# bdina9/qat-vit

Measured on AMD Instinct MI355X. Metric: images/sec QAT student step (fwd+bwd+allreduce), higher is better.
Workload: dtype f32 (emulated: int8 MFMA for grid x grid products; forward float operands as fp16 hi+lo pairs; backward gradients as ONE fp16 plane scaled per tensor - 2^-12 per element, <= 4e-4 relative L2 per stage against the fp32 reference, bf16-pair fallback on overflow; fp32 / exact-integer accumulate)

## Files before the change

include/qatvit.h:

```cpp
#ifndef QATVIT_H
#define QATVIT_H

#include <stdint.h>

#ifdef __cplusplus
extern "C" {
#endif
#if defined(__GNUC__) || defined(__clang__)
#pragma GCC visibility push(default)
#endif

#define QATVIT_ABI_VERSION 4

int qatvit_abi_version(void);
const char* qatvit_last_error(void);
const char* qatvit_target_arch(void);

int64_t qatvit_fq_workspace_bytes(int64_t channels);
int qatvit_fq_forward(const float* x, float* y, uint8_t* mask_bits,
                      float* running_min, float* running_max, float* scale, int32_t* zero_point,
                      const int64_t* observer_on, const int64_t* fake_quant_on,
                      float averaging_const, int32_t qmin, int32_t qmax,
                      int64_t channels, int64_t inner, int32_t per_channel, int32_t symmetric,
                      void* workspace, void* stream);
// ... 75 lines not shown
    const void* P; const void* Q; const uint32_t* lut; const float* s1; const float* s2; float* C; const float* W; const float* w_scale; const int32_t* w_zp; float* dbias;
    const float* row_div; int32_t N, Kw, ldp, ldq, ldc;
};
int64_t qatvit_gemm_tn_stream_scratch_bytes(void);
int qatvit_gemm_tn_stream_dy16(int32_t mode, const struct qatvit_tn_item* items, int32_t n, int32_t M, int32_t center, int32_t w_per_channel, int32_t w_qmin, int32_t w_qmax,
                               float* scratch, int64_t scratch_bytes, void* stream);

int32_t qatvit_attn_padded_tokens(int32_t T);
int qatvit_attn_forward(const float* qkv, const float* qp, int32_t qmin, int32_t qmax, int32_t B, int32_t T, int32_t H,
                        int32_t D, void* O_hi, void* O_lo, float* lse, void* stream);
int qatvit_attn_forward_f16(const float* qkv, const float* qp, int32_t qmin, int32_t qmax, int32_t B, int32_t T, int32_t H,
                            int32_t D, void* O_hi, void* O_lo, float* lse, void* O16_hi, void* O16_lo, float* o16_scale, void* qkv_codes,
                            void* qkv_mask, void* stream);
int qatvit_attn_backward(const float* qkv, const float* qp, int32_t qmin, int32_t qmax, int32_t B, int32_t T, int32_t H,
                         int32_t D, const void* O_hi, const void* O_lo, const float* lse, float* delta, const float* dO,
                         void* dqkv_hi, void* dqkv_lo, const float* col_scale, const void* qkv_codes, const void* qkv_mask, void* stream);
int qatvit_attn_backward_live(const float* qkv, const float* qp, int32_t qmin, int32_t qmax, int32_t B, int32_t T, int32_t H,
                              int32_t D, const void* O_hi, const void* O_lo, const float* lse, float* delta, const float* dO,
                              void* dqkv_hi, void* dqkv_lo, const float* col_scale, const void* qkv_codes, const void* qkv_mask,
                              int32_t live_q_tiles, int32_t dO_cls, void* stream);

int qatvit_rows_gather(const void* tall, void* compact, int32_t rows, int32_t T, int32_t width, int64_t stride, void* stream);
int qatvit_rows_scatter(const void* compact, void* tall, int32_t rows, int32_t T, int32_t width, void* stream);

typedef struct qatvit_cfg {
    int32_t batch, img_size, patch_size, in_chans;
    int32_t embed_dim, depth, num_heads, mlp_hidden, num_classes;
    int32_t act_qmin, act_qmax;
    int32_t w_qmin, w_qmax;
    int32_t w_per_channel;
    float averaging_const;
    float ln_eps;
} qatvit_cfg;

typedef struct qatvit_fq {
    float* min_val;
    float* max_val;
    float* scale;
    int32_t* zero_point;
    const int64_t* observer_on;
    const int64_t* fake_quant_on;
} qatvit_fq;

int32_t qatvit_student_num_params(const qatvit_cfg* cfg);
int32_t qatvit_student_num_act_fq(const qatvit_cfg* cfg);
int32_t qatvit_student_num_weight_fq(const qatvit_cfg* cfg);
// ... 127 lines not shown
```

qat-vit_amd/csrc/capi.hip:

```cpp
#include <stdarg.h>
#include <stdlib.h>
#include <string.h>

#include "../../include/qatvit.h"
#include "qv_common.h"
#include "qv_kernels.h"

namespace qv {
static thread_local char g_err[512] = "";
void set_error(const char* fmt, ...) {
    va_list ap;
    va_start(ap, fmt);
    vsnprintf(g_err, sizeof(g_err), fmt, ap);
    va_end(ap);
}

static bool knob(const char* name) {
    const char* v = getenv(name);
    return !v || atoi(v) != 0;
}
const Knobs& knobs() {
    static const Knobs k{knob("QATVIT_I8"), knob("QATVIT_F16"), knob("QATVIT_FC2_CODES"), knob("QATVIT_FC1_BITS"), knob("QATVIT_FC2W_CODES"),
                         knob("QATVIT_WBATCH"), knob("QATVIT_ATTN_CODES"), knob("QATVIT_QKV_2PASS"), knob("QATVIT_LNB_FUSE"), knob("QATVIT_QP_LATE"),
                         knob("QATVIT_TN_STREAM"), knob("QATVIT_TN_Q8"), knob("QATVIT_ATTN_BWD_FUSED"), knob("QATVIT_F16_STRIP"), knob("QATVIT_I8_STRIP"), knob("QATVIT_LN_STRIP"),
                         knob("QATVIT_CLS_BWD")};
    return k;
}
}

using namespace qv;

extern "C" {

int qatvit_abi_version(void) { return QATVIT_ABI_VERSION; }
const char* qatvit_last_error(void) { return qv::g_err; }
const char* qatvit_target_arch(void) { return "gfx950"; }

int64_t qatvit_fq_workspace_bytes(int64_t channels) {
    if (channels < 1) channels = 1;
    return channels * (2 * (int64_t)sizeof(uint32_t) + 4 * (int64_t)sizeof(float));
}

int qatvit_fq_forward(const float* x, float* y, uint8_t* mask_bits, float* running_min, float* running_max, float* scale,
                      int32_t* zero_point, const int64_t* observer_on, const int64_t* fake_quant_on, float averaging_const,
                      int32_t qmin, int32_t qmax, int64_t channels, int64_t inner, int32_t per_channel, int32_t symmetric,
                      void* workspace, void* stream) {
    QV_CHECK_ARG(x && y && running_min && running_max && scale && zero_point && observer_on && fake_quant_on && workspace,
                 "qatvit_fq_forward: null pointer argument");
// ... 443 lines not shown
                     ((uintptr_t)mix & 3) == 0 && ((uintptr_t)erase & 3) == 0,
                 "qatvit_image_batch_rrc_erase: misaligned pointer");
    if (launch_image_batch_rrc_erase(data, index, B, N, S, D, windows, table, rrc, mix, erase, out, (hipStream_t)stream)) return 1;
    QV_CHECK_LAUNCH("qatvit_image_batch_rrc_erase");
    return 0;
}

int qatvit_rows_gather(const void* tall, void* compact, int32_t rows, int32_t T, int32_t width, int64_t stride, void* stream) {
    RowMoveTab t;
    t.n = 1; t.m[0] = RowMove{tall, compact, stride, width};
    if (launch_rows_gather(t, rows, T, (hipStream_t)stream)) return 1;
    QV_CHECK_LAUNCH("qatvit_rows_gather");
    return 0;
}

int qatvit_rows_scatter(const void* compact, void* tall, int32_t rows, int32_t T, int32_t width, void* stream) {
    RowMoveTab t;
    t.n = 1; t.m[0] = RowMove{compact, tall, width, width};
    if (launch_rows_scatter(t, rows, T, (hipStream_t)stream)) return 1;
    QV_CHECK_LAUNCH("qatvit_rows_scatter");
    return 0;
}

}
```

qat-vit_amd/csrc/elt.hip:

```cpp
#include <stdlib.h>

#include <algorithm>

#include "qv_common.h"
#include "qv_device.h"
#include "qv_kernels.h"
#include "qv_qparams.h"

namespace qv {

struct QP { float s, inv, zp, on; };
__device__ inline QP load_qp(const float* qp) { return QP{qp[0], qp[1], qp[2], qp[3]}; }
__device__ inline float fqv(float x, const QP& q, float fqmin, float fqmax, bool& in) {
    const float t = rintf(x * q.inv) + q.zp;
    in = (t >= fqmin && t <= fqmax) || q.on == 0.f;
    const float y = (fminf(fmaxf(t, fqmin), fqmax) - q.zp) * q.s;
    return q.on != 0.f ? y : x;
}
__device__ inline float fqi(float x, const QP& q, float fqmin, float fqmax) {
    return fminf(fmaxf(rintf(x * q.inv) + q.zp, fqmin), fqmax) - q.zp;
}

__device__ inline void store_split4(__bf16* hi, __bf16* lo, int64_t off, float a, float b, float c, float d) {
    uint2 h, l;
// ... 412 lines not shown
    __syncthreads();
    const int lane = threadIdx.x & 63, wave = threadIdx.x >> 6;
    for (int c = wave; c < C; c += 4) {
        float acc = 0.f;
        for (int k = lane; k < D; k += 64) acc += sh[k] * (float)wq[(int64_t)c * D + k];
        acc = wave_sum(acc);
        if (lane == 0) {
            const float v = acc * (q.s * w_scale[w_per_channel ? c : 0]) + bias[c];
            logits_pre[(int64_t)b * C + c] = v;
            stat_atomic(stats, stat_slots, v, v);
        }
    }
}

__global__ void k_logits_fq(const float* __restrict__ pre, const float* __restrict__ qp, int qmin, int qmax, float* __restrict__ out, int n) {
    const QP q = load_qp(qp);
    const int i = blockIdx.x * blockDim.x + threadIdx.x;
    if (i < n) {
        bool in;
        out[i] = fqv(pre[i], q, qmin, qmax, in);
    }
}

__global__ __launch_bounds__(256) void k_head_bwd(const float* __restrict__ dlogits, const float* __restrict__ logits_pre, const float* __restrict__ qp_logits,
                                                  int qmin, int qmax, const float* __restrict__ hq, const float* __restrict__ qp_norm,
                                                  const __bf16* __restrict__ wq, const float* __restrict__ W, const float* __restrict__ w_scale,
                                                  const int32_t* __restrict__ w_zp, int w_per_channel, int w_qmin, int w_qmax,
                                                  float* __restrict__ dW, float* __restrict__ dbias, float* __restrict__ dh, int B, int D, int C) {
    const QP ql = load_qp(qp_logits);
    const int kch = (D + 63) / 64;
    if ((int)blockIdx.x < C * kch) {
        const int c = blockIdx.x / kch, k = (blockIdx.x % kch) * 64 + (threadIdx.x & 63), grp = threadIdx.x >> 6;
        const float s_norm = qp_norm[0];
        const int ci = w_per_channel ? c : 0;
        const float inv = __fdiv_rn(1.0f, w_scale[ci]), fzp = (float)w_zp[ci];
        float acc = 0.f, dbacc = 0.f;
        const int bper = (B + 3) / 4, b_lo = grp * bper, b_hi = min(B, b_lo + bper);
        if (k < D) {
            for (int b = b_lo; b < b_hi; ++b) {
                bool in;
                fqv(logits_pre[(int64_t)b * C + c], ql, qmin, qmax, in);
                const float dl = in ? dlogits[(int64_t)b * C + c] : 0.f;
                acc += dl * hq[(int64_t)b * D + k];
                dbacc += dl;
            }
        }
        __shared__ float sacc[4][64], sdb[4];
        sacc[grp][threadIdx.x & 63] = acc;
        if ((threadIdx.x & 63) == 0) sdb[grp] = dbacc;
        __syncthreads();
        if (grp == 0 && k < D) {
            const float tot = ((sacc[0][threadIdx.x] + sacc[1][threadIdx.x]) + sacc[2][threadIdx.x]) + sacc[3][threadIdx.x];
            const float t = rintf(W[(int64_t)c * D + k] * inv) + fzp;
            const bool win = t >= (float)w_qmin && t <= (float)w_qmax;
            dW[(int64_t)c * D + k] = win ? tot * s_norm : 0.f;
            if (k == 0) dbias[c] = ((sdb[0] + sdb[1]) + sdb[2]) + sdb[3];
        }
    } else {
        const int b = blockIdx.x - C * kch;
        for (int k = threadIdx.x; k < D; k += blockDim.x) {
            float acc = 0.f;
            for (int c = 0; c < C; ++c) {
                bool in;
                fqv(logits_pre[(int64_t)b * C + c], ql, qmin, qmax, in);
                const float dl = in ? dlogits[(int64_t)b * C + c] : 0.f;
                acc += dl * (float)wq[(int64_t)c * D + k] * w_scale[w_per_channel ? c : 0];
            }
            dh[(int64_t)b * D + k] = acc;
        }
    }
}

__global__ __launch_bounds__(64) void k_embed_bwd(const float* __restrict__ dx0, const float* __restrict__ Y0, const float* __restrict__ qp,
                                                  int qmin, int qmax, float* __restrict__ dpos, float* __restrict__ dcls,
                                                  __bf16* __restrict__ dY0_hi, __bf16* __restrict__ dY0_lo, int B, int T, int D) {
    const QP q = load_qp(qp);
    const int d4 = D / 4;
    const int64_t n4 = (int64_t)T * d4;
    constexpr int UNR = 16;
    for (int64_t i = blockIdx.x * (int64_t)blockDim.x + threadIdx.x; i < n4; i += (int64_t)gridDim.x * blockDim.x) {
        const int t = (int)(i / d4), c = (int)(i % d4) * 4;
        const int ty = t > 0 ? t - 1 : 0;
        float4 acc = make_float4(0.f, 0.f, 0.f, 0.f);
        for (int b0 = 0; b0 < B; b0 += UNR) {
            float4 g[UNR], y[UNR];
#pragma unroll
            for (int u = 0; u < UNR; ++u) {
                const int b = b0 + u < B ? b0 + u : B - 1;
                g[u] = *reinterpret_cast<const float4*>(dx0 + ((int64_t)b * T + t) * D + c);
                y[u] = *reinterpret_cast<const float4*>(Y0 + ((int64_t)b * (T - 1) + ty) * D + c);
            }
#pragma unroll
            for (int u = 0; u < UNR; ++u) { pin4(g[u]); pin4(y[u]); }
#pragma unroll
            for (int u = 0; u < UNR; ++u) {
                if (b0 + u < B) {
                    acc.x += g[u].x; acc.y += g[u].y; acc.z += g[u].z; acc.w += g[u].w;
                    if (t > 0) {
                        bool i0, i1, i2, i3;
                        fqv(y[u].x, q, qmin, qmax, i0); fqv(y[u].y, q, qmin, qmax, i1); fqv(y[u].z, q, qmin, qmax, i2); fqv(y[u].w, q, qmin, qmax, i3);
                        store_split4(dY0_hi, dY0_lo, ((int64_t)(b0 + u) * (T - 1) + (t - 1)) * D + c, i0 ? g[u].x : 0.f, i1 ? g[u].y : 0.f,
                                     i2 ? g[u].z : 0.f, i3 ? g[u].w : 0.f);
                    }
                }
            }
        }
        *reinterpret_cast<float4*>(dpos + (int64_t)t * D + c) = acc;
        if (t == 0) *reinterpret_cast<float4*>(dcls + c) = acc;
    }
}

__device__ inline void wquant_body(const float* __restrict__ W, const float* __restrict__ qp, int per_channel, int qmin, int qmax,
                                   __bf16* __restrict__ wq, __bf16* __restrict__ wqT, int N, int K, int bx, int by,
                                   int8_t* __restrict__ w8 = nullptr, int32_t* __restrict__ wsum = nullptr, _Float16* __restrict__ w16 = nullptr,
                                   int8_t* __restrict__ w8f = nullptr, int64_t wT16_gap = 0,
                                   bool wT16_frag = false) {
    __shared__ float tile[32][33];
    const int tx = threadIdx.x & 31, ty = threadIdx.x >> 5;
    const int n0 = by * 32, k0 = bx * 32;
#pragma unroll
    for (int i = 0; i < 4; ++i) {
        const int n = n0 + ty + 8 * i, k = k0 + tx;
        float v = 0.f;
        if (n < N && k < K) {
            const QP q = load_qp(qp + 4 * (per_channel ? n : 0));
            v = q.on != 0.f ? fqi(W[(int64_t)n * K + k], q, qmin, qmax) : W[(int64_t)n * K + k];
            wq[(int64_t)n * K + k] = (__bf16)v;
            if (w8) w8[(int64_t)n * K + k] = (int8_t)v;
            if (w16) w16[(int64_t)n * K + k] = (_Float16)v;
            if (w8f) w8f[w8f_offset(n, k, K)] = (int8_t)v;
        }
// ... 11 lines not shown
        char* const wT16f = (wT16_gap && wT16_frag) ? reinterpret_cast<char*>(wqT) + 2 * wT16_gap : nullptr;
#pragma unroll
        for (int i = 0; i < 4; ++i) {
            const int k = k0 + ty + 8 * i, n = n0 + tx;
            if (n < N && k < K) {
                wqT[(int64_t)k * N + n] = (__bf16)tile[tx][ty + 8 * i];
                if (wT16) wT16[(int64_t)k * N + n] = (_Float16)tile[tx][ty + 8 * i];
                if (wT16f) *reinterpret_cast<_Float16*>(wT16f + w8f_offset(k, 2 * n, 2 * N)) = (_Float16)tile[tx][ty + 8 * i];
            }
        }
    }
}
__global__ __launch_bounds__(256) void k_wquant(const float* __restrict__ W, const float* __restrict__ qp, int per_channel, int qmin, int qmax,
                                                __bf16* __restrict__ wq, __bf16* __restrict__ wqT, int N, int K) {
    wquant_body(W, qp, per_channel, qmin, qmax, wq, wqT, N, K, blockIdx.x, blockIdx.y);
}
__global__ __launch_bounds__(256) void k_w_quant_all(const WQuantTab t) {
    int wi = 0;
    while (wi + 1 < t.n && (int)blockIdx.x >= t.blk0[wi + 1]) ++wi;
    const int b = blockIdx.x - t.blk0[wi], kt = (t.K[wi] + 31) / 32;
    wquant_body(t.W[wi], t.qp[wi], t.per_channel, t.qmin, t.qmax, reinterpret_cast<__bf16*>(t.wq[wi]), reinterpret_cast<__bf16*>(t.wqT[wi]), t.N[wi],
                t.K[wi], b % kt, b / kt, reinterpret_cast<int8_t*>(t.w8[wi]), t.wsum[wi], reinterpret_cast<_Float16*>(t.w16[wi]),
                reinterpret_cast<int8_t*>(t.w8f[wi]), t.wT16 ? wT16_gap_bytes(t.N[wi], t.K[wi]) : 0, ((t.wT16f_mask >> wi) & 1ull) != 0);
}
static_assert(sizeof(WQuantTab) <= 4096, "WQuantTab travels as a kernel argument");
__global__ __launch_bounds__(256) void k_w8_fragment_order(const int8_t* __restrict__ B8, int8_t* __restrict__ B8f, int N, int K) {
    const int64_t i = blockIdx.x * (int64_t)blockDim.x + threadIdx.x;
    if (i >= (int64_t)N * K) return;
    B8f[w8f_offset((int)(i / K), (int)(i % K), K)] = B8[i];
}
int launch_w8_fragment_order(const void* B8, void* B8f, int N, int K, hipStream_t st) {
    if (N < 48 || N % 48 != 0 || K % 64 != 0 || !B8 || !B8f) { set_error("w8_fragment_order: need N %% 48 == 0, K %% 64 == 0 (N=%d K=%d)", N, K); return 1; }
    k_w8_fragment_order<<<cdiv((int64_t)N * K, 256), 256, 0, st>>>(reinterpret_cast<const int8_t*>(B8), reinterpret_cast<int8_t*>(B8f), N, K);
    return 0;
}

int launch_img_patches(const float* img, void* out_bf16, const float* qp, int qmin, int qmax, int B, int C, int H, int W, int P, hipStream_t st,
                       void* out8, int center) {
    if (P % 8 != 0 || H % P != 0 || W % P != 0) { set_error("img_patches: patch %d must be a multiple of 8 and divide %dx%d", P, H, W); return 1; }
    const int64_t n8 = (int64_t)B * C * H * W / 8;
    k_img_patches<<<flat_grid(n8), 256, 0, st>>>(img, reinterpret_cast<__bf16*>(out_bf16), qp, qmin, qmax, B, C, H, W, P, reinterpret_cast<int8_t*>(out8),
                                                 center);
    return 0;
}

int launch_resid_fq_lnstats(int mode, const float* x_prev, const float* Y, const float* qpY, int qmin, int qmax, const float* cls, const float* pos,
// ... 72 lines not shown
    const int nv = (D + 255) / 256;
    if (acc) { if (nv == 1) QV_LNB(1, 1); else if (nv == 2) QV_LNB(1, 2); else QV_LNB(1, 3); }
    else { if (nv == 1) QV_LNB(0, 1); else if (nv == 2) QV_LNB(0, 2); else QV_LNB(0, 3); }
#undef QV_LNB
    return 0;
}

int launch_head_fwd(const float* x, const float* mean, const float* rstd, const float* gamma, const float* beta, const float* qp_norm, int qmin,
                    int qmax, const void* wq, const float* w_scale, int w_per_channel, const float* bias, float* hq, float* logits_pre,
                    uint32_t* stats, int stat_slots, int B, int D, int T, int C, hipStream_t st) {
    k_head_fwd<<<B, 256, D * sizeof(float), st>>>(x, mean, rstd, gamma, beta, qp_norm, qmin, qmax, reinterpret_cast<const __bf16*>(wq), w_scale,
                                                   w_per_channel, bias, hq, logits_pre, stats, stat_slots, D, T, C);
    return 0;
}

int launch_logits_fq(const float* pre, const float* qp, int qmin, int qmax, float* out, int n, hipStream_t st) {
    k_logits_fq<<<cdiv(n, 256), 256, 0, st>>>(pre, qp, qmin, qmax, out, n);
    return 0;
}

int launch_head_bwd(const float* dlogits, const float* logits_pre, const float* qp_logits, int qmin, int qmax, const float* hq, const float* qp_norm,
                    const void* wq, const float* W, const float* w_scale, const int32_t* w_zp, int w_per_channel, int w_qmin, int w_qmax, float* dW,
                    float* dbias, float* dh, int B, int D, int C, hipStream_t st) {
    k_head_bwd<<<C * ((D + 63) / 64) + B, 256, 0, st>>>(dlogits, logits_pre, qp_logits, qmin, qmax, hq, qp_norm, reinterpret_cast<const __bf16*>(wq), W, w_scale, w_zp,
                                      w_per_channel, w_qmin, w_qmax, dW, dbias, dh, B, D, C);
    return 0;
}

int launch_embed_bwd(const float* dx0, const float* Y0, const float* qp, int qmin, int qmax, float* dpos, float* dcls, void* dY0_hi, void* dY0_lo,
                     int B, int T, int D, hipStream_t st) {
    k_embed_bwd<<<(int)cdiv((int64_t)T * (D / 4), 64), 64, 0, st>>>(dx0, Y0, qp, qmin, qmax, dpos, dcls, reinterpret_cast<__bf16*>(dY0_hi),
                                                                  reinterpret_cast<__bf16*>(dY0_lo), B, T, D);
    return 0;
}

__global__ void k_zero_i32(int32_t* p, int64_t n) {
    for (int64_t i = blockIdx.x * (int64_t)blockDim.x + threadIdx.x; i < n; i += (int64_t)gridDim.x * blockDim.x) p[i] = 0;
}
int launch_zero_i32(int32_t* p, int64_t n, hipStream_t st) {
    k_zero_i32<<<(int)cdiv(n, 256) > 1024 ? 1024 : (int)cdiv(n, 256), 256, 0, st>>>(p, n);
    return 0;
}
__global__ __launch_bounds__(256) void k_rows_gather(const RowMoveTab t, int rows, int T) {
    const RowMove m = t.m[blockIdx.y];
    const int wpr = m.width / 4;
    const int64_t tall = (int64_t)T * (m.stride / 4);
    const uint32_t* __restrict__ src = reinterpret_cast<const uint32_t*>(m.src);
    uint32_t* __restrict__ dst = reinterpret_cast<uint32_t*>(m.dst);
    const int total = rows * wpr;
    for (int i = blockIdx.x * 256 + threadIdx.x; i < total; i += gridDim.x * 256) {
        const int b = i / wpr, j = i - b * wpr;
        dst[i] = src[b * tall + j];
    }
}
// ... 18 lines not shown
        const int unit = scatter ? 16 : 4;
        const bool ok = m.src && m.dst && m.width >= unit && m.width % unit == 0 && m.stride % unit == 0 && (scatter ? m.stride == m.width : m.stride >= m.width) &&
                        (int64_t)rows * (scatter ? T : 1) * (m.width / unit) < (1ll << 31) &&
                        (reinterpret_cast<uintptr_t>(m.src) | reinterpret_cast<uintptr_t>(m.dst)) % unit == 0;
        if (!ok) { set_error("%s: tensor %d: width %d, stride %lld (bytes; need %% %d == 0%s, aligned bases, < 2^31 units)", who, k, m.width, (long long)m.stride, unit,
                             scatter ? " and stride == width" : ""); return 1; }
    }
    return 0;
}
int launch_rows_gather(const RowMoveTab& t, int rows, int T, hipStream_t st) {
    if (rows_check("rows_gather", t, rows, T, false)) return 1;
    int64_t most = 0;
    for (int k = 0; k < t.n; ++k) most = std::max<int64_t>(most, (int64_t)rows * (t.m[k].width / 4));
    k_rows_gather<<<dim3(std::min(cdiv(most, 256), 512), t.n), 256, 0, st>>>(t, rows, T);
    return 0;
}
int launch_rows_scatter(const RowMoveTab& t, int rows, int T, hipStream_t st) {
    if (rows_check("rows_scatter", t, rows, T, true)) return 1;
    int64_t most = 0;
    for (int k = 0; k < t.n; ++k) most = std::max<int64_t>(most, (int64_t)rows * T * (t.m[k].width / 16));
    k_rows_scatter<<<dim3(std::min(cdiv(most, 256 * 4), 4096), t.n), 256, 0, st>>>(t, rows, T);
    return 0;
}
int launch_w_quant_all(WQuantTab& t, hipStream_t st) {
    int b = 0;
    for (int i = 0; i < t.n; ++i) {
        t.blk0[i] = b;
        b += (int)(cdiv(t.K[i], 32) * cdiv(t.N[i], 32));
    }
    t.blk0[t.n] = b;
    k_w_quant_all<<<b, 256, 0, st>>>(t);
    return 0;
}
int launch_wquant(const float* W, const float* qp, int per_channel, int qmin, int qmax, void* wq, void* wqT, int N, int K, hipStream_t st) {
    dim3 grid(cdiv(K, 32), cdiv(N, 32));
    k_wquant<<<grid, 256, 0, st>>>(W, qp, per_channel, qmin, qmax, reinterpret_cast<__bf16*>(wq), reinterpret_cast<__bf16*>(wqT), N, K);
    return 0;
}

}
```

qat-vit_amd/csrc/qv_common.h:

```cpp
#pragma once
#include <hip/hip_runtime.h>
#include <stdint.h>
#include <stdio.h>

namespace qv {

constexpr int kWave = 64;

void set_error(const char* fmt, ...);

struct Knobs {
    bool i8;
    bool f16;
    bool fc2_codes;
    bool fc1_bits;
    bool fc2w_codes;
    bool wbatch;
    bool attn_codes;
    bool qkv_2pass;
    bool lnb_fuse;
    bool qp_late;
    bool tn_stream;
    bool tn_q8;
    bool attn_bwd_fused;
    bool f16_strip;
    bool i8_strip;
    bool ln_strip;
    bool cls_bwd;
};
const Knobs& knobs();

#define QV_CHECK_ARG(cond, ...)                 \
    do {                                        \
        if (!(cond)) {                          \
            qv::set_error(__VA_ARGS__);         \
            return 1;                           \
        }                                       \
    } while (0)

#define QV_CHECK_LAUNCH(name)                                                     \
    do {                                                                          \
        hipError_t e_ = hipGetLastError();                                        \
        if (e_ != hipSuccess) {                                                   \
            qv::set_error("%s: launch failed: %s", name, hipGetErrorString(e_));  \
            return 2;                                                             \
        }                                                                         \
    } while (0)

__host__ __device__ inline uint32_t f2ord(float f) {
    uint32_t u = __builtin_bit_cast(uint32_t, f);
// ... 80 lines not shown
```

qat-vit_amd/csrc/qv_kernels.h:

```cpp
#pragma once
#include <hip/hip_runtime.h>
#include <stdint.h>

namespace qv {

int launch_fq_forward(const float* x, float* y, uint8_t* mask_bits, float* running_min, float* running_max, float* scale,
                      int32_t* zero_point, const int64_t* observer_on, const int64_t* fake_quant_on, float c, int qmin, int qmax,
                      int64_t channels, int64_t inner, bool per_channel, bool symmetric, void* workspace, hipStream_t st);
int launch_fq_backward(const float* dy, const uint8_t* mask_bits, float* dx, int64_t n, hipStream_t st);

int launch_ln_forward(const float* x, const float* gamma, const float* beta, float* y, float* mean, float* rstd, int64_t rows,
                      int64_t dim, float eps, hipStream_t st);
int launch_ln_backward(const float* dy, const float* x, const float* gamma, const float* mean, const float* rstd, float* dx,
                       float* dgamma, float* dbeta, int64_t rows, int64_t dim, hipStream_t st);

int launch_kd_ce_loss(const float* student, const float* teacher, const int64_t* labels, int64_t batch, int64_t classes, float kd_temp,
                      float kd_alpha, float label_smoothing, float* out3, float* dlogits, hipStream_t st);
int launch_kd_ce_loss_table(const float* student, const float* table, int64_t table_rows, const int64_t* index, const int64_t* labels, int64_t batch,
                            int64_t classes, float kd_temp, float kd_alpha, float label_smoothing, float* out3, float* dlogits, hipStream_t st);
int launch_kd_ce_loss_mix(const float* student, const float* teacher, const float* table, int64_t table_rows, const int64_t* index,
                          const int64_t* labels, const int32_t* mix, int64_t batch, int64_t classes, float kd_temp, float kd_alpha,
                          float label_smoothing, float* out3, float* dlogits, hipStream_t st);

int launch_minmax(const float* x, int64_t channels, int64_t inner, int per_channel, uint32_t* ws, int nslots, hipStream_t st);
// ... 131 lines not shown
int launch_logits_fq(const float* pre, const float* qp, int qmin, int qmax, float* out, int n, hipStream_t st);
int launch_head_bwd(const float* dlogits, const float* logits_pre, const float* qp_logits, int qmin, int qmax, const float* hq, const float* qp_norm,
                    const void* wq, const float* W, const float* w_scale, const int32_t* w_zp, int w_per_channel, int w_qmin, int w_qmax, float* dW,
                    float* dbias, float* dh, int B, int D, int C, hipStream_t st);
int launch_embed_bwd(const float* dx0, const float* Y0, const float* qp, int qmin, int qmax, float* dpos, float* dcls, void* dY0_hi, void* dY0_lo,
                     int B, int T, int D, hipStream_t st);
constexpr int kMaxW = 52;
struct WObsTab { const float* W[kMaxW]; uint32_t* ws[kMaxW]; int N[kMaxW], K[kMaxW], blk0[kMaxW + 1]; int n, per_channel, nslots; };
struct WQpTab {
    uint32_t* ws[kMaxW]; float* rmin[kMaxW]; float* rmax[kMaxW]; float* scale[kMaxW]; int32_t* zp[kMaxW]; float* qp[kMaxW];
    const int64_t* obs_on[kMaxW]; const int64_t* fq_on[kMaxW]; int N[kMaxW], blk0[kMaxW + 1]; int n, per_channel, nslots, qmin, qmax; float c;
};
struct WQuantTab {
    const float* W[kMaxW]; const float* qp[kMaxW]; void* wq[kMaxW]; void* wqT[kMaxW]; void* w8[kMaxW]; int32_t* wsum[kMaxW];
    void* w16[kMaxW];
    void* w8f[kMaxW];
    int N[kMaxW], K[kMaxW], blk0[kMaxW + 1]; int n, per_channel, qmin, qmax;
    int wT16;
    unsigned long long wT16f_mask;
};
__host__ __device__ inline int64_t wT16_gap_bytes(int N, int K) { return ((int64_t)N * K * 2 + 255) & ~(int64_t)255; }
int launch_w_observe_all(WObsTab& t, hipStream_t st);
int launch_w_qparams_all(WQpTab& t, hipStream_t st);
int launch_w_quant_all(WQuantTab& t, hipStream_t st);
int launch_zero_i32(int32_t* p, int64_t n, hipStream_t st);
struct ObsFoldEntry {
    uint32_t* ws; float* rmin; float* rmax; float* scale; int32_t* zp; const int64_t* obs_on; const int64_t* fq_on;
    int32_t channels, nslots, symmetric, qmin, qmax, blk0;
};
int launch_obs_fold(const ObsFoldEntry* tab, int n, int nblocks, float c, hipStream_t st);
int launch_wquant(const float* W, const float* qp, int per_channel, int qmin, int qmax, void* wq, void* wqT, int N, int K, hipStream_t st);

constexpr int kDyHdrWords = 64, kDySlotWords = 256, kDyAmaxStride = 32, kDyAmaxSlots = 8;
inline int64_t dy16_state_bytes(int nslots) { return 4ll * (kDyHdrWords + (int64_t)nslots * kDySlotWords); }
int launch_dy16_begin(uint32_t* state, int nslots, const float* dlogits, int n_dlogits, hipStream_t st);
int launch_dy16_set_mirror(uint32_t* state, void* host_pinned, hipStream_t st);
int launch_dy16_end(uint32_t* state, int nslots, int check_overflow, hipStream_t st);
int launch_absmax_bf16(const void* hi, int64_t n, uint32_t* amax, hipStream_t st);
int launch_q8_to_bf16int(const void* q8, const float* qp, int center, void* plane, int64_t n, hipStream_t st);
int launch_f16int_to_bf16int(void* plane, int64_t n, hipStream_t st);

int attn_padded_tokens(int T);
int launch_attn_fwd(const float* qkv, const float* qp, int qmin, int qmax, int B, int T, int H, int D, void* O_hi, void* O_lo, float* lse,
                    hipStream_t st, void* O16_hi = nullptr, void* O16_lo = nullptr, float* o16_scale = nullptr, void* codes = nullptr,
                    void* cmask = nullptr);
int launch_attn_bwd(const float* qkv, const float* qp, int qmin, int qmax, int B, int T, int H, int D, const void* O_hi, const void* O_lo,
                    const float* lse, float* delta, const float* dO, void* dqkv_hi, void* dqkv_lo, const float* col_scale, hipStream_t st,
// ... 65 lines not shown
```

qat-vit_amd/native.py:

```python
from __future__ import annotations

import ctypes
import os
import subprocess
from ctypes import c_char_p, c_double, c_float, c_int, c_int32, c_int64, c_void_p

_HERE = os.path.dirname(os.path.abspath(__file__))
LIB_PATH = os.path.join(_HERE, "libqatvit.so")
CSRC = os.path.join(_HERE, "csrc")
_lib = None

SIGNATURES = {
    "qatvit_abi_version": (c_int, []),
    "qatvit_last_error": (c_char_p, []),
    "qatvit_target_arch": (c_char_p, []),
    "qatvit_fq_workspace_bytes": (c_int64, [c_int64]),
    "qatvit_fq_forward": (c_int, [c_void_p] * 9 + [c_float, c_int32, c_int32, c_int64, c_int64, c_int32, c_int32, c_void_p, c_void_p]),
    "qatvit_fq_backward": (c_int, [c_void_p, c_void_p, c_void_p, c_int64, c_void_p]),
    "qatvit_ln_forward": (c_int, [c_void_p] * 6 + [c_int64, c_int64, c_float, c_void_p]),
    "qatvit_ln_backward": (c_int, [c_void_p] * 8 + [c_int64, c_int64, c_void_p]),
    "qatvit_kd_ce_loss": (c_int, [c_void_p, c_void_p, c_void_p, c_int64, c_int64, c_float, c_float, c_float, c_void_p, c_void_p, c_void_p]),
    "qatvit_kd_ce_loss_table": (c_int, [c_void_p, c_void_p, c_int64, c_void_p, c_void_p, c_int64, c_int64, c_float, c_float, c_float, c_void_p, c_void_p, c_void_p]),
    "qatvit_kd_ce_loss_mix": (c_int, [c_void_p, c_void_p, c_void_p, c_int64, c_void_p, c_void_p, c_void_p, c_int64, c_int64, c_float, c_float, c_float,
                                      c_void_p, c_void_p, c_void_p]),
# ... 3 lines not shown
    "qatvit_optim_adamw_ema": (c_int, [c_void_p] * 8 + [c_int32, c_int64] + [c_double] * 5 + [c_int64, c_double, c_void_p, c_void_p]),
    "qatvit_optim_adamw_groups_ema": (c_int, [c_void_p] * 9 + [c_int32, c_int64, c_void_p, c_int32, c_double, c_void_p, c_void_p]),
    "qatvit_optim_ema": (c_int, [c_void_p] * 5 + [c_int32, c_int64, c_double, c_void_p]),
    "qatvit_optim_swap": (c_int, [c_void_p] * 5 + [c_int32, c_int64, c_void_p]),
    "qatvit_gemm_nt": (c_int, [c_void_p] * 4 + [c_int32] * 6 + [c_void_p] * 6),
    "qatvit_gemm_nt_f16": (c_int, [c_void_p] * 4 + [c_int32] * 6 + [c_void_p] * 6),
    "qatvit_gemm_nt_i8_minmax": (c_int, [c_void_p] * 4 + [c_int32] * 6 + [c_void_p] * 6),
    "qatvit_w8_fragment_order": (c_int, [c_void_p, c_void_p, c_int32, c_int32, c_void_p]),
    "qatvit_i8_strip": (c_int, [c_int32] + [c_void_p] * 4 + [c_int32] * 5 + [c_void_p] * 6 + [c_int32, c_int32, c_void_p, c_void_p, c_int32] + [c_void_p] * 4),
    "qatvit_ln_apply_quant8": (c_int, [c_void_p] * 6 + [c_int32, c_int32, c_void_p, c_int32, c_int64, c_int32, c_void_p]),
    "qatvit_i8_strip_ln": (c_int, [c_void_p] * 5 + [c_int32, c_int32] + [c_void_p] * 4 + [c_int32] * 5 + [c_void_p] * 5),
    "qatvit_gemm_nt_codes": (c_int, [c_void_p] * 4 + [c_int32] * 6 + [c_void_p] * 6),
    "qatvit_gemm_nt_i8": (c_int, [c_void_p] * 4 + [c_int32, c_void_p] + [c_int32] * 6 + [c_void_p] * 6),
    "qatvit_gemm_tn_scratch_bytes": (c_int64, []),
    "qatvit_gemm_tn": (c_int, [c_void_p] * 5 + [c_int32] * 6 + [c_void_p] * 4 + [c_int32] * 3 + [c_void_p] * 3 + [c_int64, c_void_p]),
    "qatvit_gemm_tn_codes": (c_int, [c_void_p] * 5 + [c_int32] * 6 + [c_void_p] * 4 + [c_int32] * 3 + [c_void_p] * 3 + [c_int64, c_void_p]),
    "qatvit_gemm_nt_dy16": (c_int, [c_void_p] * 3 + [c_int32] * 6 + [c_void_p] * 3),
    "qatvit_gemm_tn_dy16": (c_int, [c_void_p] * 6 + [c_int32] * 6 + [c_void_p] * 5 + [c_int32] * 3 + [c_void_p] * 3 + [c_int64, c_void_p]),
    "qatvit_gemm_tn_q8_dy16": (c_int, [c_void_p] * 3 + [c_int32, c_void_p] + [c_int32] * 6 + [c_void_p] * 4 + [c_int32] * 3 + [c_void_p] * 3 + [c_int64, c_void_p]),
    "qatvit_gemm_tn_stream_scratch_bytes": (c_int64, []),
    "qatvit_gemm_tn_stream_dy16": (c_int, [c_int32, c_void_p, c_int32, c_int32, c_int32, c_int32, c_int32, c_int32, c_void_p, c_int64, c_void_p]),
    "qatvit_rows_gather": (c_int, [c_void_p, c_void_p, c_int32, c_int32, c_int32, c_int64, c_void_p]),
    "qatvit_rows_scatter": (c_int, [c_void_p, c_void_p, c_int32, c_int32, c_int32, c_void_p]),
    "qatvit_attn_padded_tokens": (c_int32, [c_int32]),
    "qatvit_attn_forward": (c_int, [c_void_p, c_void_p] + [c_int32] * 6 + [c_void_p] * 4),
    "qatvit_attn_forward_f16": (c_int, [c_void_p, c_void_p] + [c_int32] * 6 + [c_void_p] * 9),
    "qatvit_attn_backward": (c_int, [c_void_p, c_void_p] + [c_int32] * 6 + [c_void_p] * 11),
    "qatvit_attn_backward_live": (c_int, [c_void_p, c_void_p] + [c_int32] * 6 + [c_void_p] * 10 + [c_int32, c_int32, c_void_p]),
    "qatvit_student_num_params": (c_int32, [c_void_p]),
    "qatvit_student_num_act_fq": (c_int32, [c_void_p]),
    "qatvit_student_num_weight_fq": (c_int32, [c_void_p]),
    "qatvit_student_workspace_bytes": (c_int64, [c_void_p]),
    "qatvit_student_init": (c_int, [c_void_p, c_void_p, c_void_p]),
    "qatvit_student_forward": (c_int, [c_void_p] * 8),
    "qatvit_student_backward": (c_int, [c_void_p] * 7 + [c_int32, c_int32, c_void_p]),
    "qatvit_student_forward_stages": (c_int, [c_void_p] * 7 + [c_int32, c_int32, c_int32, c_void_p]),
    "qatvit_student_forward_part": (c_int, [c_void_p] * 5 + [c_int32, c_int32, c_int32, c_void_p]),
    "qatvit_student_backward_stages": (c_int, [c_void_p] * 7 + [c_int32, c_int32, c_int32, c_void_p]),
    "qatvit_student_tensor_offset": (c_int64, [c_void_p, c_char_p, c_int32]),
    "qatvit_student_dy16_supported": (c_int32, [c_void_p]),
    "qatvit_student_ln_in_strip": (c_int32, [c_void_p, c_int32]),
    "qatvit_student_dy16_to_pair": (c_int, [c_void_p, c_void_p, c_void_p]),
    "qatvit_student_dy16_set_mirror": (c_int, [c_void_p, c_void_p, c_void_p, c_void_p]),
    "qatvit_teacher_workspace_bytes": (c_int64, [c_void_p]),
    "qatvit_teacher_forward": (c_int, [c_void_p] * 8),
    "qatvit_teacher_forward_f16": (c_int, [c_void_p, c_void_p, c_void_p, c_int32, c_void_p, c_void_p, c_void_p, c_void_p]),
# ... 132 lines not shown
```

Baseline: 16640.

## Split batch reductions across thread groups and add vectorized weight-quant kernel

The head-backward kernel now splits its batch reduction across 16 wave groups instead of 4 and unrolls the per-sample loads by four. The embed-backward kernel splits the batch across 8 groups per 32 items and combines the partial sums in shared memory, which gives more parallelism along B. A new vectorized weight-quantization kernel handles 64x64 tiles with float4 loads, 16-byte stores and a shared-memory transpose for wqT; it is enabled by default when K%64==0 and all pointers are 16-byte aligned. New C API entry points expose these kernels for testing, and the wider reductions change the floating-point summation order.

```diff
diff --git a/include/qatvit.h b/include/qatvit.h
--- a/include/qatvit.h
+++ b/include/qatvit.h
@@ -121,6 +121,14 @@
 
 int qatvit_rows_gather(const void* tall, void* compact, int32_t rows, int32_t T, int32_t width, int64_t stride, void* stream);
 int qatvit_rows_scatter(const void* compact, void* tall, int32_t rows, int32_t T, int32_t width, void* stream);
+
+int qatvit_w_quant(const float* W, const float* qp, int32_t per_channel, int32_t qmin, int32_t qmax, void* wq, void* wqT, void* w8, int32_t* wsum, void* w16,
+                   void* w8f, int32_t wT16, int32_t wT16f, int32_t N, int32_t K, int32_t vec, void* stream);
+int qatvit_embed_bwd(const float* dx0, const float* Y0, const float* qp, int32_t qmin, int32_t qmax, float* dpos, float* dcls, void* dY0_hi, void* dY0_lo,
+                     int32_t B, int32_t T, int32_t D, void* stream);
+int qatvit_head_bwd(const float* dlogits, const float* logits_pre, const float* qp_logits, int32_t qmin, int32_t qmax, const float* hq, const float* qp_norm,
+                    const void* wq, const float* W, const float* w_scale, const int32_t* w_zp, int32_t w_per_channel, int32_t w_qmin, int32_t w_qmax,
+                    float* dW, float* dbias, float* dh, int32_t B, int32_t D, int32_t C, void* stream);
 
 typedef struct qatvit_cfg {
     int32_t batch, img_size, patch_size, in_chans;
diff --git a/qat-vit_amd/csrc/capi.hip b/qat-vit_amd/csrc/capi.hip
--- a/qat-vit_amd/csrc/capi.hip
+++ b/qat-vit_amd/csrc/capi.hip
@@ -23,7 +23,7 @@
     static const Knobs k{knob("QATVIT_I8"), knob("QATVIT_F16"), knob("QATVIT_FC2_CODES"), knob("QATVIT_FC1_BITS"), knob("QATVIT_FC2W_CODES"),
                          knob("QATVIT_WBATCH"), knob("QATVIT_ATTN_CODES"), knob("QATVIT_QKV_2PASS"), knob("QATVIT_LNB_FUSE"), knob("QATVIT_QP_LATE"),
                          knob("QATVIT_TN_STREAM"), knob("QATVIT_TN_Q8"), knob("QATVIT_ATTN_BWD_FUSED"), knob("QATVIT_F16_STRIP"), knob("QATVIT_I8_STRIP"), knob("QATVIT_LN_STRIP"),
-                         knob("QATVIT_CLS_BWD")};
+                         knob("QATVIT_WQUANT_VEC"), knob("QATVIT_CLS_BWD")};
     return k;
 }
 }
@@ -513,4 +513,41 @@
     return 0;
 }
 
-}
+int qatvit_w_quant(const float* W, const float* qp, int32_t per_channel, int32_t qmin, int32_t qmax, void* wq, void* wqT, void* w8, int32_t* wsum, void* w16,
+                   void* w8f, int32_t wT16, int32_t wT16f, int32_t N, int32_t K, int32_t vec, void* stream) {
+    QV_CHECK_ARG(W && qp && wq, "qatvit_w_quant: null pointer argument");
+    QV_CHECK_ARG(N >= 1 && K >= 1 && qmin < qmax, "qatvit_w_quant: N=%d K=%d qmin=%d qmax=%d", N, K, qmin, qmax);
+    QV_CHECK_ARG(!w8f || (N % 48 == 0 && K % 64 == 0), "qatvit_w_quant: the fragment order of w8f needs N %% 48 == 0, K %% 64 == 0 (N=%d K=%d)", N, K);
+    QV_CHECK_ARG(!wT16 || wqT, "qatvit_w_quant: wT16 follows wqT");
+    QV_CHECK_ARG(!wT16f || (wT16 && K % 48 == 0 && N % 32 == 0), "qatvit_w_quant: wT16f follows wT16 and needs K %% 48 == 0, N %% 32 == 0 (N=%d K=%d)", N, K);
+    WQuantTab t{};
+    t.n = 1; t.per_channel = per_channel; t.qmin = qmin; t.qmax = qmax; t.wT16 = wT16; t.wT16f_mask = wT16f ? 1ull : 0ull;
+    t.W[0] = W; t.qp[0] = qp; t.wq[0] = wq; t.wqT[0] = wqT; t.w8[0] = w8; t.wsum[0] = wsum; t.w16[0] = w16; t.w8f[0] = w8f; t.N[0] = N; t.K[0] = K;
+    if (launch_w_quant_all(t, (hipStream_t)stream, vec)) return 1;
+    QV_CHECK_LAUNCH("qatvit_w_quant");
+    return 0;
+}
+
+int qatvit_embed_bwd(const float* dx0, const float* Y0, const float* qp, int32_t qmin, int32_t qmax, float* dpos, float* dcls, void* dY0_hi, void* dY0_lo,
+                     int32_t B, int32_t T, int32_t D, void* stream) {
+    QV_CHECK_ARG(dx0 && Y0 && qp && dpos && dcls && dY0_hi && dY0_lo, "qatvit_embed_bwd: null pointer argument");
+    QV_CHECK_ARG(B >= 1 && T >= 2 && D >= 4 && D % 4 == 0, "qatvit_embed_bwd: B=%d T=%d D=%d (need T >= 2, D %% 4 == 0)", B, T, D);
+    QV_CHECK_ARG((((uintptr_t)dx0 | (uintptr_t)Y0 | (uintptr_t)dpos | (uintptr_t)dcls) & 15) == 0 && (((uintptr_t)dY0_hi | (uintptr_t)dY0_lo) & 7) == 0,
+                 "qatvit_embed_bwd: misaligned pointer");
+    if (launch_embed_bwd(dx0, Y0, qp, qmin, qmax, dpos, dcls, dY0_hi, dY0_lo, B, T, D, (hipStream_t)stream)) return 1;
+    QV_CHECK_LAUNCH("qatvit_embed_bwd");
+    return 0;
+}
+
+int qatvit_head_bwd(const float* dlogits, const float* logits_pre, const float* qp_logits, int32_t qmin, int32_t qmax, const float* hq, const float* qp_norm,
+                    const void* wq, const float* W, const float* w_scale, const int32_t* w_zp, int32_t w_per_channel, int32_t w_qmin, int32_t w_qmax,
+                    float* dW, float* dbias, float* dh, int32_t B, int32_t D, int32_t C, void* stream) {
+    QV_CHECK_ARG(dlogits && logits_pre && qp_logits && hq && qp_norm && wq && W && w_scale && w_zp && dW && dbias && dh, "qatvit_head_bwd: null pointer argument");
+    QV_CHECK_ARG(B >= 1 && D >= 1 && C >= 1, "qatvit_head_bwd: B=%d D=%d C=%d", B, D, C);
+    if (launch_head_bwd(dlogits, logits_pre, qp_logits, qmin, qmax, hq, qp_norm, wq, W, w_scale, w_zp, w_per_channel, w_qmin, w_qmax, dW, dbias, dh, B, D, C,
+                        (hipStream_t)stream)) return 1;
+    QV_CHECK_LAUNCH("qatvit_head_bwd");
+    return 0;
+}
+
+}
diff --git a/qat-vit_amd/csrc/elt.hip b/qat-vit_amd/csrc/elt.hip
--- a/qat-vit_amd/csrc/elt.hip
+++ b/qat-vit_amd/csrc/elt.hip
@@ -458,7 +458,8 @@
     }
 }
 
-__global__ __launch_bounds__(256) void k_head_bwd(const float* __restrict__ dlogits, const float* __restrict__ logits_pre, const float* __restrict__ qp_logits,
+constexpr int kHeadGroups = 16;
+__global__ __launch_bounds__(64 * kHeadGroups) void k_head_bwd(const float* __restrict__ dlogits, const float* __restrict__ logits_pre, const float* __restrict__ qp_logits,
                                                   int qmin, int qmax, const float* __restrict__ hq, const float* __restrict__ qp_norm,
                                                   const __bf16* __restrict__ wq, const float* __restrict__ W, const float* __restrict__ w_scale,
                                                   const int32_t* __restrict__ w_zp, int w_per_channel, int w_qmin, int w_qmax,
@@ -471,26 +472,41 @@
         const int ci = w_per_channel ? c : 0;
         const float inv = __fdiv_rn(1.0f, w_scale[ci]), fzp = (float)w_zp[ci];
         float acc = 0.f, dbacc = 0.f;
-        const int bper = (B + 3) / 4, b_lo = grp * bper, b_hi = min(B, b_lo + bper);
+        const int bper = (B + kHeadGroups - 1) / kHeadGroups, b_lo = min(B, grp * bper), b_hi = min(B, b_lo + bper);
         if (k < D) {
-            for (int b = b_lo; b < b_hi; ++b) {
-                bool in;
-                fqv(logits_pre[(int64_t)b * C + c], ql, qmin, qmax, in);
-                const float dl = in ? dlogits[(int64_t)b * C + c] : 0.f;
-                acc += dl * hq[(int64_t)b * D + k];
-                dbacc += dl;
-            }
-        }
-        __shared__ float sacc[4][64], sdb[4];
+            for (int b0 = b_lo; b0 < b_hi; b0 += 4) {
+                float lp[4], dg[4], h[4];
+#pragma unroll
+                for (int u = 0; u < 4; ++u) {
+                    const int b = b0 + u < b_hi ? b0 + u : b_hi - 1;
+                    lp[u] = logits_pre[(int64_t)b * C + c];
+                    dg[u] = dlogits[(int64_t)b * C + c];
+                    h[u] = hq[(int64_t)b * D + k];
+                }
+#pragma unroll
+                for (int u = 0; u < 4; ++u) {
+                    if (b0 + u < b_hi) {
+                        bool in;
+                        fqv(lp[u], ql, qmin, qmax, in);
+                        const float dl = in ? dg[u] : 0.f;
+                        acc += dl * h[u];
+                        dbacc += dl;
+                    }
+                }
+            }
+        }
+        __shared__ float sacc[kHeadGroups][64], sdb[kHeadGroups];
         sacc[grp][threadIdx.x & 63] = acc;
         if ((threadIdx.x & 63) == 0) sdb[grp] = dbacc;
         __syncthreads();
         if (grp == 0 && k < D) {
-            const float tot = ((sacc[0][threadIdx.x] + sacc[1][threadIdx.x]) + sacc[2][threadIdx.x]) + sacc[3][threadIdx.x];
+            float tot = sacc[0][threadIdx.x], db = sdb[0];
+#pragma unroll
+            for (int g = 1; g < kHeadGroups; ++g) { tot += sacc[g][threadIdx.x]; db += sdb[g]; }
             const float t = rintf(W[(int64_t)c * D + k] * inv) + fzp;
             const bool win = t >= (float)w_qmin && t <= (float)w_qmax;
             dW[(int64_t)c * D + k] = win ? tot * s_norm : 0.f;
-            if (k == 0) dbias[c] = ((sdb[0] + sdb[1]) + sdb[2]) + sdb[3];
+            if (k == 0) dbias[c] = db;
         }
     } else {
         const int b = blockIdx.x - C * kch;
@@ -507,22 +523,26 @@
     }
 }
 
-__global__ __launch_bounds__(64) void k_embed_bwd(const float* __restrict__ dx0, const float* __restrict__ Y0, const float* __restrict__ qp,
-                                                  int qmin, int qmax, float* __restrict__ dpos, float* __restrict__ dcls,
-                                                  __bf16* __restrict__ dY0_hi, __bf16* __restrict__ dY0_lo, int B, int T, int D) {
+constexpr int kEmbItems = 32, kEmbGroups = 8;
+__global__ __launch_bounds__(kEmbItems * kEmbGroups) void k_embed_bwd(const float* __restrict__ dx0, const float* __restrict__ Y0, const float* __restrict__ qp,
+                                                                      int qmin, int qmax, float* __restrict__ dpos, float* __restrict__ dcls,
+                                                                      __bf16* __restrict__ dY0_hi, __bf16* __restrict__ dY0_lo, int B, int T, int D) {
     const QP q = load_qp(qp);
     const int d4 = D / 4;
     const int64_t n4 = (int64_t)T * d4;
-    constexpr int UNR = 16;
-    for (int64_t i = blockIdx.x * (int64_t)blockDim.x + threadIdx.x; i < n4; i += (int64_t)gridDim.x * blockDim.x) {
-        const int t = (int)(i / d4), c = (int)(i % d4) * 4;
-        const int ty = t > 0 ? t - 1 : 0;
-        float4 acc = make_float4(0.f, 0.f, 0.f, 0.f);
-        for (int b0 = 0; b0 < B; b0 += UNR) {
+    constexpr int UNR = 8;
+    const int item = threadIdx.x % kEmbItems, grp = threadIdx.x / kEmbItems;
+    const int bper = (B + kEmbGroups - 1) / kEmbGroups, b_lo = min(B, grp * bper), b_hi = min(B, b_lo + bper);
+    const int64_t i = blockIdx.x * (int64_t)kEmbItems + item;
+    const int t = (int)(i / d4), c = (int)(i % d4) * 4;
+    const int ty = t > 0 ? t - 1 : 0;
+    float4 acc = make_float4(0.f, 0.f, 0.f, 0.f);
+    if (i < n4) {
+        for (int b0 = b_lo; b0 < b_hi; b0 += UNR) {
             float4 g[UNR], y[UNR];
 #pragma unroll
             for (int u = 0; u < UNR; ++u) {
-                const int b = b0 + u < B ? b0 + u : B - 1;
+                const int b = b0 + u < b_hi ? b0 + u : b_hi - 1;
                 g[u] = *reinterpret_cast<const float4*>(dx0 + ((int64_t)b * T + t) * D + c);
                 y[u] = *reinterpret_cast<const float4*>(Y0 + ((int64_t)b * (T - 1) + ty) * D + c);
             }
@@ -530,7 +550,7 @@
             for (int u = 0; u < UNR; ++u) { pin4(g[u]); pin4(y[u]); }
 #pragma unroll
             for (int u = 0; u < UNR; ++u) {
-                if (b0 + u < B) {
+                if (b0 + u < b_hi) {
                     acc.x += g[u].x; acc.y += g[u].y; acc.z += g[u].z; acc.w += g[u].w;
                     if (t > 0) {
                         bool i0, i1, i2, i3;
@@ -541,8 +561,16 @@
                 }
             }
         }
-        *reinterpret_cast<float4*>(dpos + (int64_t)t * D + c) = acc;
-        if (t == 0) *reinterpret_cast<float4*>(dcls + c) = acc;
+    }
+    __shared__ float4 part[kEmbGroups][kEmbItems];
+    part[grp][item] = acc;
+    __syncthreads();
+    if (grp == 0 && i < n4) {
+        float4 s = part[0][item];
+#pragma unroll
+        for (int k = 1; k < kEmbGroups; ++k) { const float4 a = part[k][item]; s.x += a.x; s.y += a.y; s.z += a.z; s.w += a.w; }
+        *reinterpret_cast<float4*>(dpos + (int64_t)t * D + c) = s;
+        if (t == 0) *reinterpret_cast<float4*>(dcls + c) = s;
     }
 }
 
@@ -600,6 +628,92 @@
     wquant_body(t.W[wi], t.qp[wi], t.per_channel, t.qmin, t.qmax, reinterpret_cast<__bf16*>(t.wq[wi]), reinterpret_cast<__bf16*>(t.wqT[wi]), t.N[wi],
                 t.K[wi], b % kt, b / kt, reinterpret_cast<int8_t*>(t.w8[wi]), t.wsum[wi], reinterpret_cast<_Float16*>(t.w16[wi]),
                 reinterpret_cast<int8_t*>(t.w8f[wi]), t.wT16 ? wT16_gap_bytes(t.N[wi], t.K[wi]) : 0, ((t.wT16f_mask >> wi) & 1ull) != 0);
+}
+__global__ __launch_bounds__(256) void k_w_quant_all_vec(const WQuantTab t) {
+    int wi = 0;
+    while (wi + 1 < t.n && (int)blockIdx.x >= t.blk0[wi + 1]) ++wi;
+    const int N = t.N[wi], K = t.K[wi];
+    const int b = blockIdx.x - t.blk0[wi], kt = K / 64;
+    const int n0 = (b / kt) * 64, k0 = (b % kt) * 64;
+    const float* __restrict__ W = t.W[wi];
+    __bf16* __restrict__ wq = reinterpret_cast<__bf16*>(t.wq[wi]);
+    __bf16* __restrict__ wqT = reinterpret_cast<__bf16*>(t.wqT[wi]);
+    int8_t* __restrict__ w8 = reinterpret_cast<int8_t*>(t.w8[wi]);
+    int8_t* __restrict__ w8f = reinterpret_cast<int8_t*>(t.w8f[wi]);
+    _Float16* __restrict__ w16 = reinterpret_cast<_Float16*>(t.w16[wi]);
+    int32_t* __restrict__ wsum = t.wsum[wi];
+    __shared__ float tile[64][65];
+    {
+        const int r = threadIdx.x >> 2, kq = (threadIdx.x & 3) * 16, n = n0 + r;
+        float v[16];
+#pragma unroll
+        for (int j = 0; j < 16; ++j) v[j] = 0.f;
+        if (n < N) {
+            const QP q = load_qp(t.qp[wi] + 4 * (t.per_channel ? n : 0));
+            const int64_t o = (int64_t)n * K + k0 + kq;
+            float4 a[4];
+#pragma unroll
+            for (int j = 0; j < 4; ++j) a[j] = *reinterpret_cast<const float4*>(W + o + 4 * j);
+#pragma unroll
+            for (int j = 0; j < 4; ++j) { v[4 * j] = a[j].x; v[4 * j + 1] = a[j].y; v[4 * j + 2] = a[j].z; v[4 * j + 3] = a[j].w; }
+            if (q.on != 0.f) {
+#pragma unroll
+                for (int j = 0; j < 16; ++j) v[j] = fqi(v[j], q, t.qmin, t.qmax);
+            }
+            bf16x8 ob[2];
+            f16x8 oh[2];
+            int8_t o8[16];
+#pragma unroll
+            for (int j = 0; j < 16; ++j) { ob[j / 8][j % 8] = (__bf16)v[j]; oh[j / 8][j % 8] = (_Float16)v[j]; o8[j] = (int8_t)v[j]; }
+            uint4 p8;
+            __builtin_memcpy(&p8, o8, 16);
+            *reinterpret_cast<bf16x8*>(wq + o) = ob[0];
+            *reinterpret_cast<bf16x8*>(wq + o + 8) = ob[1];
+            if (w8) *reinterpret_cast<uint4*>(w8 + o) = p8;
+            if (w16) { *reinterpret_cast<f16x8*>(w16 + o) = oh[0]; *reinterpret_cast<f16x8*>(w16 + o + 8) = oh[1]; }
+            if (w8f) *reinterpret_cast<uint4*>(w8f + w8f_offset(n, k0 + kq, K)) = p8;
+        }
+#pragma unroll
+        for (int j = 0; j < 16; ++j) tile[r][kq + j] = v[j];
+    }
+    __syncthreads();
+    if (wsum && threadIdx.x < 64 && n0 + (int)threadIdx.x < N) {
+        float s0 = 0.f, s1 = 0.f;
+#pragma unroll
+        for (int k = 0; k < 32; ++k) { s0 += tile[threadIdx.x][k]; s1 += tile[threadIdx.x][32 + k]; }
+        atomicAdd(&wsum[n0 + threadIdx.x], (int)s0 + (int)s1);
+    }
+    if (!wqT) return;
+    const int64_t gap = t.wT16 ? wT16_gap_bytes(N, K) : 0;
+    _Float16* const wT16 = gap ? reinterpret_cast<_Float16*>(reinterpret_cast<char*>(wqT) + gap) : nullptr;
+    char* const wT16f = (gap && ((t.wT16f_mask >> wi) & 1ull) != 0) ? reinterpret_cast<char*>(wqT) + 2 * gap : nullptr;
+    if (N % 8 == 0) {
+#pragma unroll
+        for (int i = 0; i < 2; ++i) {
+            const int p = i * 256 + threadIdx.x, kk = p >> 3, nn = (p & 7) * 8;
+            const int k = k0 + kk, n = n0 + nn;
+            if (n < N) {
+                bf16x8 ob;
+                f16x8 oh;
+#pragma unroll
+                for (int j = 0; j < 8; ++j) { const float v = tile[nn + j][kk]; ob[j] = (__bf16)v; oh[j] = (_Float16)v; }
+                *reinterpret_cast<bf16x8*>(wqT + (int64_t)k * N + n) = ob;
+                if (wT16) *reinterpret_cast<f16x8*>(wT16 + (int64_t)k * N + n) = oh;
+                if (wT16f) *reinterpret_cast<f16x8*>(wT16f + w8f_offset(k, 2 * n, 2 * N)) = oh;
+            }
+        }
+    } else {
+        for (int e = threadIdx.x; e < 64 * 64; e += 256) {
+            const int kk = e >> 6, nn = e & 63;
+            const int k = k0 + kk, n = n0 + nn;
+            if (n < N) {
+                const float v = tile[nn][kk];
+                wqT[(int64_t)k * N + n] = (__bf16)v;
+                if (wT16) wT16[(int64_t)k * N + n] = (_Float16)v;
+                if (wT16f) *reinterpret_cast<_Float16*>(wT16f + w8f_offset(k, 2 * n, 2 * N)) = (_Float16)v;
+            }
+        }
+    }
 }
 static_assert(sizeof(WQuantTab) <= 4096, "WQuantTab travels as a kernel argument");
 __global__ __launch_bounds__(256) void k_w8_fragment_order(const int8_t* __restrict__ B8, int8_t* __restrict__ B8f, int N, int K) {
@@ -718,14 +832,14 @@
 int launch_head_bwd(const float* dlogits, const float* logits_pre, const float* qp_logits, int qmin, int qmax, const float* hq, const float* qp_norm,
                     const void* wq, const float* W, const float* w_scale, const int32_t* w_zp, int w_per_channel, int w_qmin, int w_qmax, float* dW,
                     float* dbias, float* dh, int B, int D, int C, hipStream_t st) {
-    k_head_bwd<<<C * ((D + 63) / 64) + B, 256, 0, st>>>(dlogits, logits_pre, qp_logits, qmin, qmax, hq, qp_norm, reinterpret_cast<const __bf16*>(wq), W, w_scale, w_zp,
+    k_head_bwd<<<C * ((D + 63) / 64) + B, 64 * kHeadGroups, 0, st>>>(dlogits, logits_pre, qp_logits, qmin, qmax, hq, qp_norm, reinterpret_cast<const __bf16*>(wq), W, w_scale, w_zp,
                                       w_per_channel, w_qmin, w_qmax, dW, dbias, dh, B, D, C);
     return 0;
 }
 
 int launch_embed_bwd(const float* dx0, const float* Y0, const float* qp, int qmin, int qmax, float* dpos, float* dcls, void* dY0_hi, void* dY0_lo,
                      int B, int T, int D, hipStream_t st) {
-    k_embed_bwd<<<(int)cdiv((int64_t)T * (D / 4), 64), 64, 0, st>>>(dx0, Y0, qp, qmin, qmax, dpos, dcls, reinterpret_cast<__bf16*>(dY0_hi),
+    k_embed_bwd<<<(int)cdiv((int64_t)T * (D / 4), kEmbItems), kEmbItems * kEmbGroups, 0, st>>>(dx0, Y0, qp, qmin, qmax, dpos, dcls, reinterpret_cast<__bf16*>(dY0_hi),
                                                                   reinterpret_cast<__bf16*>(dY0_lo), B, T, D);
     return 0;
 }
@@ -790,7 +904,23 @@
     k_rows_scatter<<<dim3(std::min(cdiv(most, 256 * 4), 4096), t.n), 256, 0, st>>>(t, rows, T);
     return 0;
 }
-int launch_w_quant_all(WQuantTab& t, hipStream_t st) {
+int launch_w_quant_all(WQuantTab& t, hipStream_t st, int vec) {
+    bool v = vec < 0 ? knobs().wquant_vec : vec != 0;
+    for (int i = 0; i < t.n && v; ++i) {
+        const uintptr_t a = reinterpret_cast<uintptr_t>(t.W[i]) | reinterpret_cast<uintptr_t>(t.wq[i]) | reinterpret_cast<uintptr_t>(t.wqT[i]) |
+                            reinterpret_cast<uintptr_t>(t.w8[i]) | reinterpret_cast<uintptr_t>(t.w16[i]) | reinterpret_cast<uintptr_t>(t.w8f[i]);
+        v = t.K[i] % 64 == 0 && a % 16 == 0;
+    }
+    if (v) {
+        int b = 0;
+        for (int i = 0; i < t.n; ++i) {
+            t.blk0[i] = b;
+            b += (t.K[i] / 64) * cdiv(t.N[i], 64);
+        }
+        t.blk0[t.n] = b;
+        k_w_quant_all_vec<<<b, 256, 0, st>>>(t);
+        return 0;
+    }
     int b = 0;
     for (int i = 0; i < t.n; ++i) {
         t.blk0[i] = b;
diff --git a/qat-vit_amd/csrc/qv_common.h b/qat-vit_amd/csrc/qv_common.h
--- a/qat-vit_amd/csrc/qv_common.h
+++ b/qat-vit_amd/csrc/qv_common.h
@@ -26,6 +26,7 @@
     bool f16_strip;
     bool i8_strip;
     bool ln_strip;
+    bool wquant_vec;
     bool cls_bwd;
 };
 const Knobs& knobs();
diff --git a/qat-vit_amd/csrc/qv_kernels.h b/qat-vit_amd/csrc/qv_kernels.h
--- a/qat-vit_amd/csrc/qv_kernels.h
+++ b/qat-vit_amd/csrc/qv_kernels.h
@@ -177,7 +177,7 @@
 __host__ __device__ inline int64_t wT16_gap_bytes(int N, int K) { return ((int64_t)N * K * 2 + 255) & ~(int64_t)255; }
 int launch_w_observe_all(WObsTab& t, hipStream_t st);
 int launch_w_qparams_all(WQpTab& t, hipStream_t st);
-int launch_w_quant_all(WQuantTab& t, hipStream_t st);
+int launch_w_quant_all(WQuantTab& t, hipStream_t st, int vec = -1);
 int launch_zero_i32(int32_t* p, int64_t n, hipStream_t st);
 struct ObsFoldEntry {
     uint32_t* ws; float* rmin; float* rmax; float* scale; int32_t* zp; const int64_t* obs_on; const int64_t* fq_on;
diff --git a/qat-vit_amd/native.py b/qat-vit_amd/native.py
--- a/qat-vit_amd/native.py
+++ b/qat-vit_amd/native.py
@@ -49,6 +49,9 @@
     "qatvit_gemm_tn_stream_dy16": (c_int, [c_int32, c_void_p, c_int32, c_int32, c_int32, c_int32, c_int32, c_int32, c_void_p, c_int64, c_void_p]),
     "qatvit_rows_gather": (c_int, [c_void_p, c_void_p, c_int32, c_int32, c_int32, c_int64, c_void_p]),
     "qatvit_rows_scatter": (c_int, [c_void_p, c_void_p, c_int32, c_int32, c_int32, c_void_p]),
+    "qatvit_w_quant": (c_int, [c_void_p, c_void_p, c_int32, c_int32, c_int32] + [c_void_p] * 6 + [c_int32] * 5 + [c_void_p]),
+    "qatvit_embed_bwd": (c_int, [c_void_p] * 3 + [c_int32, c_int32] + [c_void_p] * 4 + [c_int32] * 3 + [c_void_p]),
+    "qatvit_head_bwd": (c_int, [c_void_p] * 3 + [c_int32, c_int32] + [c_void_p] * 6 + [c_int32] * 3 + [c_void_p] * 3 + [c_int32] * 3 + [c_void_p]),
     "qatvit_attn_padded_tokens": (c_int32, [c_int32]),
     "qatvit_attn_forward": (c_int, [c_void_p, c_void_p] + [c_int32] * 6 + [c_void_p] * 4),
     "qatvit_attn_forward_f16": (c_int, [c_void_p, c_void_p] + [c_int32] * 6 + [c_void_p] * 9),
```

After: 16730 (median of 6 runs). No clear change (+0.5%).
